# pySTEPS/pysteps

Measured on AMD Instinct MI355X. Metric: Mpixels*leadsteps/s (LK+semilag) at 4096x4096 fp32, higher is better.
Workload: dtype f32

## Files before the change

### pysteps_amd/csrc/lk.hip

```cpp
#include <algorithm>
#include <cmath>
#include <cstring>
#include <functional>
#include <vector>

#include "common.h"

#pragma clang fp contract(off)

namespace psh {
namespace {

enum Stat : int {
  kMinAll = 0,
  kNanCount,
  kMaxAll,
  kMinFeat,
  kMaxFeat,
  kEigMax,
  kNumStats = 8
};

constexpr int kRedBlocks = 1024;

// ... 333 lines not shown
    unsigned char t[4], f[4];
#pragma unroll
    for (int j = 0; j < 4; ++j) {
      const size_t p = i + j;
      float v = p < npx ? clean[p] : fill;
      const bool ok = isfinite(v);
      if (!ok) v = fill;
      t[j] = quantise(v, fill, hi);
      f[j] = quantise((ok && p >= first_feature_px) ? v : fill, flo, fhi);
    }
    if (i + 3 < npx && (npx & 3) == 0) {
      *reinterpret_cast<uchar4 *>(trk + i) = make_uchar4(t[0], t[1], t[2], t[3]);
      if (feat) *reinterpret_cast<uchar4 *>(feat + i) = make_uchar4(f[0], f[1], f[2], f[3]);
    } else {
      for (int j = 0; j < 4 && i + j < npx; ++j) {
        trk[i + j] = t[j];
        if (feat) feat[i + j] = f[j];
      }
    }
  }
}

constexpr int kU8Rows = 4;
template <bool VEC>
__global__ __launch_bounds__(256) void lk_to_u8_bits(const float *__restrict__ img,
                                                     const unsigned long long *__restrict__ keepbits, int nstrips,
                                                     int m, int n, int buffer_mask, float *__restrict__ stats,
                                                     unsigned char *__restrict__ trk, unsigned char *__restrict__ feat,
                                                     const unsigned *__restrict__ slots) {
  const float fill = stats[kMinAll], hi = slots_max(slots, kSlMaxAll);
  const float flo = slots_min(slots, kSlMinFeat), fhi = slots_max(slots, kSlMaxFeat);
  if (blockIdx.x == 0 && blockIdx.y == 0 && threadIdx.x == 0) {
    stats[kMaxAll] = hi;
    stats[kMinFeat] = flo;
    stats[kMaxFeat] = fhi;
  }
  const int first_row = buffer_mask > 0 ? (stats[kNanCount] > 0.f ? 2 : 1) : 0;
  const bool same_scale = flo == fill && fhi == hi;
  const int x = (blockIdx.x * 256 + threadIdx.x) * 4;
  const int y0 = blockIdx.y * kU8Rows;
  if (x >= n) return;
  const int strip = x / kOpenColsW, shift = x - strip * kOpenColsW + 2;
  float v[kU8Rows][4];
  unsigned long long w[kU8Rows];
#pragma unroll
  for (int r = 0; r < kU8Rows; ++r) {
    const int y = min(y0 + r, m - 1);
    const float *row = img + static_cast<size_t>(y) * n + x;
    w[r] = keepbits[static_cast<size_t>(y) * nstrips + strip];
    if (VEC) {
      const float4 q = *reinterpret_cast<const float4 *>(row);
      v[r][0] = q.x, v[r][1] = q.y, v[r][2] = q.z, v[r][3] = q.w;
    } else {
#pragma unroll
      for (int j = 0; j < 4; ++j) v[r][j] = x + j < n ? row[j] : 0.f;
    }
  }
#pragma unroll
  for (int r = 0; r < kU8Rows; ++r) {
    const int y = y0 + r;
    if (y >= m) break;
    const unsigned keep = static_cast<unsigned>(w[r] >> shift);
    unsigned t = 0, f = 0;
#pragma unroll
    for (int j = 0; j < 4; ++j) {
      const bool k = (keep >> j) & 1u;
      const float val = k ? v[r][j] : fill;
      t |= static_cast<unsigned>(quantise(val, fill, hi)) << (8 * j);
      if (!same_scale) f |= static_cast<unsigned>(quantise(y >= first_row ? val : fill, flo, fhi)) << (8 * j);
    }
    if (same_scale) f = y >= first_row ? t : 0u;
    const size_t at = static_cast<size_t>(y) * n + x;
    if (VEC) {
      *reinterpret_cast<unsigned *>(trk + at) = t;
      if (feat) *reinterpret_cast<unsigned *>(feat + at) = f;
    } else {
#pragma unroll
      for (int j = 0; j < 4; ++j) {
        if (x + j >= n) break;
        trk[at + j] = static_cast<unsigned char>(t >> (8 * j));
        if (feat) feat[at + j] = static_cast<unsigned char>(f >> (8 * j));
      }
    }
  }
}

__device__ __forceinline__ double wave_min_d(double v) {
#pragma unroll
  for (int d = 32; d >= 1; d >>= 1) v = fmin(v, __shfl_xor(v, d));
  return v;
}
__device__ __forceinline__ double wave_max_d(double v) {
#pragma unroll
  for (int d = 32; d >= 1; d >>= 1) v = fmax(v, __shfl_xor(v, d));
  return v;
}

__global__ __launch_bounds__(256) void lk_stats1_f64(const double *__restrict__ img, size_t npx,
                                                     double *__restrict__ partial) {
  double mn = INFINITY, bad = 0.0;
  const size_t stride = static_cast<size_t>(gridDim.x) * blockDim.x;
  for (size_t i = static_cast<size_t>(blockIdx.x) * blockDim.x + threadIdx.x; i < npx; i += stride) {
    const double v = img[i];
    const bool fin = isfinite(v);
    mn = fmin(mn, fin ? v : INFINITY);
    bad += fin ? 0.0 : 1.0;
  }
  __shared__ double s[2][4];
  mn = wave_min_d(mn);
#pragma unroll
  for (int d = 32; d >= 1; d >>= 1) bad += __shfl_xor(bad, d);
  if ((threadIdx.x & 63) == 0) {
    s[0][threadIdx.x >> 6] = mn;
    s[1][threadIdx.x >> 6] = bad;
  }
  __syncthreads();
  if (threadIdx.x == 0) {
    partial[blockIdx.x] = fmin(fmin(s[0][0], s[0][1]), fmin(s[0][2], s[0][3]));
    partial[gridDim.x + blockIdx.x] = s[1][0] + s[1][1] + s[1][2] + s[1][3];
  }
}

__global__ __launch_bounds__(kFinalThreads) void lk_final_f64(const double *__restrict__ partial, int nb, int what,
                                                             float *__restrict__ stats, double *__restrict__ dstats) {
  __shared__ double sm[3][16];
  double a = what == 0 ? INFINITY : -INFINITY, b = what == 0 ? 0.0 : INFINITY, c = -INFINITY;
  for (int i = threadIdx.x; i < nb; i += blockDim.x) {
    if (what == 0) {
      a = fmin(a, partial[i]);
      b += partial[nb + i];
    } else {
      a = fmax(a, partial[i]);
      b = fmin(b, partial[nb + i]);
      c = fmax(c, partial[2 * nb + i]);
    }
  }
  if (what == 0) {
    a = wave_min_d(a);
#pragma unroll
    for (int d = 32; d >= 1; d >>= 1) b += __shfl_xor(b, d);
  } else {
    a = wave_max_d(a);
    b = wave_min_d(b);
    c = wave_max_d(c);
  }
  const int wave = threadIdx.x >> 6, nwaves = blockDim.x >> 6;
  if ((threadIdx.x & 63) == 0) {
    sm[0][wave] = a;
    sm[1][wave] = b;
    sm[2][wave] = c;
  }
  __syncthreads();
  if (threadIdx.x == 0) {
    for (int w = 1; w < nwaves; ++w) {
      if (what == 0) {
        a = fmin(a, sm[0][w]);
        b += sm[1][w];
      } else {
        a = fmax(a, sm[0][w]);
        b = fmin(b, sm[1][w]);
        c = fmax(c, sm[2][w]);
      }
    }
    if (what == 0) {
      dstats[0] = a;
      stats[kMinAll] = static_cast<float>(a);
      stats[kNanCount] = static_cast<float>(b);
    } else {
      dstats[1] = a;
      dstats[2] = b;
      dstats[3] = c;
      stats[kMaxAll] = static_cast<float>(a);
      stats[kMinFeat] = static_cast<float>(b);
      stats[kMaxFeat] = static_cast<float>(c);
    }
  }
}

__global__ __launch_bounds__(256) void lk_open_bits_f64(const double *__restrict__ img, int m, int n,
                                                        int size_opening, int buffer_mask,
                                                        const float *__restrict__ stats,
                                                        const double *__restrict__ dstats,
                                                        float *__restrict__ clean32, double *__restrict__ clean64,
                                                        double *__restrict__ partial) {
  __shared__ double red[3][4];
  const double mn = dstats[0];
  const int lane = threadIdx.x & 63, wave = threadIdx.x >> 6;
  const int x = blockIdx.x * kOpenColsW - 2 + lane;
  const int yb = blockIdx.y * kOpenRowsWG + wave * kOpenRowsW;
  const bool col_in = x >= 0 && x < n;
  constexpr int kLoad = kOpenRowsW + 4;
  double v[kLoad];
#pragma unroll
  for (int q = 0; q < kLoad; ++q) {
    const int y = yb - 2 + q;
    v[q] = (col_in && y >= 0 && y < m) ? img[static_cast<size_t>(y) * n + x] : 0.0;
  }
  unsigned long long A[kLoad], F[kLoad];
#pragma unroll
  for (int q = 0; q < kLoad; ++q) {
    const int y = yb - 2 + q;
    const bool row_in = y >= 0 && y < m;
    F[q] = __ballot(row_in && col_in && isfinite(v[q]) && v[q] > mn);
    A[q] = F[q] | __ballot(!(row_in && col_in));
  }
  unsigned long long E[kLoad];
#pragma unroll
  for (int q = 1; q < kLoad - 1; ++q) E[q] = F[q] & (A[q] << 1) & (A[q] >> 1) & A[q - 1] & A[q + 1];
  double mx_all = -INFINITY, mn_feat = INFINITY, mx_feat = -INFINITY;
  const int first_row = buffer_mask > 0 ? (stats[kNanCount] > 0.f ? 2 : 1) : 0;
  const bool writer = lane >= 2 && lane < 2 + kOpenColsW && col_in;
#pragma unroll
  for (int q = 2; q < kLoad - 2; ++q) {
    const int y = yb - 2 + q;
    if (y >= m) break;
    const unsigned long long O = E[q] | (E[q] << 1) | (E[q] >> 1) | E[q - 1] | E[q + 1];
    double val = v[q];
    if (size_opening > 0 && ((F[q] >> lane) & 1ull) && !((O >> lane) & 1ull)) val = mn;
    if (writer) {
      if (isfinite(val)) {
        mx_all = fmax(mx_all, val);
        if (y >= first_row) {
          mn_feat = fmin(mn_feat, val);
          mx_feat = fmax(mx_feat, val);
        }
      }
      clean64[static_cast<size_t>(y) * n + x] = val;
      clean32[static_cast<size_t>(y) * n + x] = static_cast<float>(val);
    }
  }
  mx_all = wave_max_d(mx_all);
  mn_feat = wave_min_d(mn_feat);
  mx_feat = wave_max_d(mx_feat);
  if (lane == 0) {
    red[0][wave] = mx_all;
    red[1][wave] = mn_feat;
    red[2][wave] = mx_feat;
  }
  __syncthreads();
  if (threadIdx.x == 0) {
    const int b = blockIdx.y * gridDim.x + blockIdx.x, nb = gridDim.x * gridDim.y;
    partial[b] = fmax(fmax(red[0][0], red[0][1]), fmax(red[0][2], red[0][3]));
    partial[nb + b] = fmin(fmin(red[1][0], red[1][1]), fmin(red[1][2], red[1][3]));
    partial[2 * nb + b] = fmax(fmax(red[2][0], red[2][1]), fmax(red[2][2], red[2][3]));
  }
}

__device__ __forceinline__ unsigned char quantise_f64(double v, double lo, double hi) {
  const double s = (hi - lo) > 1e-8 ? (v - lo) / (hi - lo) * 255.0 : v - lo;
  return static_cast<unsigned char>(static_cast<int>(s));
}

__global__ __launch_bounds__(256) void lk_to_u8_f64(const double *__restrict__ clean, int m, int n, int buffer_mask,
                                                    const float *__restrict__ stats,
                                                    const double *__restrict__ dstats,
                                                    unsigned char *__restrict__ trk, unsigned char *__restrict__ feat) {
  const double fill = dstats[0], hi = dstats[1], flo = dstats[2], fhi = dstats[3];
  const int first_row = buffer_mask > 0 ? (stats[kNanCount] > 0.f ? 2 : 1) : 0;
  const size_t npx = static_cast<size_t>(m) * n;
  const size_t first_feature_px = static_cast<size_t>(first_row) * n;
  const size_t stride = static_cast<size_t>(gridDim.x) * blockDim.x;
  for (size_t p = static_cast<size_t>(blockIdx.x) * blockDim.x + threadIdx.x; p < npx; p += stride) {
    double v = clean[p];
    const bool ok = isfinite(v);
    if (!ok) v = fill;
    trk[p] = quantise_f64(v, fill, hi);
    if (feat) feat[p] = quantise_f64((ok && p >= first_feature_px) ? v : fill, flo, fhi);
  }
}

constexpr int kMaxBlockR = 3;

__device__ __forceinline__ bool px_allowed(const float *__restrict__ clean, int m, int n, int x,
                                           int y, int bm, bool any_nan) {
  if (!any_nan) return true;
  if (bm <= 0) return isfinite(clean[static_cast<size_t>(y) * n + x]);
  const int a = bm / 2;
  for (int j = 0; j < bm; ++j) {
    const int yy = y + j - a;
    if (yy < 0 || yy >= m) continue;
    for (int i = 0; i < bm; ++i) {
      const int xx = x + i - a;
      if (xx < 0 || xx >= n) continue;
      if (!isfinite(clean[static_cast<size_t>(yy) * n + xx])) return false;
    }
  }
  return true;
}

__device__ __forceinline__ float next_lane_f(float v) {
  return __int_as_float(__builtin_amdgcn_update_dpp(0, __float_as_int(v), 0x130 , 0xf, 0xf, true));
}
__device__ __forceinline__ double next_lane_d(double v) {
  const int lo = __builtin_amdgcn_update_dpp(0, __double2loint(v), 0x130, 0xf, 0xf, true);
  const int hi = __builtin_amdgcn_update_dpp(0, __double2hiint(v), 0x130, 0xf, 0xf, true);
  return __hiloint2double(hi, lo);
}
__device__ __forceinline__ bool walk_mirrored(int i, int n) {
  if (i >= 0 && i + 1 < n) return false;
  return reflect101(i + 1, n) != reflect101(reflect101(i, n) + 1, n);
}

constexpr int crn_cols(int block_size) { return 64 - 2 * (block_size / 2 + 1); }

template <int BS, int ROWS>
__global__ __launch_bounds__(256) void lk_corner_response_cols(
    const unsigned char *__restrict__ u8, const float *__restrict__ clean, int m, int n,
    int buffer_mask, const float *__restrict__ stats, float *__restrict__ eig,
    float *__restrict__ partial, Band band, unsigned *__restrict__ slots, int *__restrict__ zero_a, int count_a,
    int *__restrict__ zero_b, int count_b) {
  constexpr int r = BS / 2, H = r + 1, W = crn_cols(BS);
  if (blockIdx.x == 0 && blockIdx.y == 0) {
    for (int i = threadIdx.x; i < count_a; i += 256) zero_a[i] = 0;
    for (int i = threadIdx.x; i < count_b; i += 256) zero_b[i] = 0;
  }
  __shared__ float red[4];
  const int lane = threadIdx.x & 63, wave = __builtin_amdgcn_readfirstlane(threadIdx.x >> 6);
  const int x0 = blockIdx.x * W;
  const int yb = (blockIdx.y * 4 + wave) * ROWS;
  float best = 0.f;
  if (yb < m) {
    const float s = 1.0f / (4.0f * static_cast<float>(BS) * 255.0f), s2 = 2.f * s;
    const int xl = x0 - H + lane;
    const bool neg_x = walk_mirrored(xl + 1, n);
    const float sx = neg_x ? -s : s, sx2 = neg_x ? -s2 : s2;
    const unsigned char *col = u8 + reflect101(xl, n);
    const bool few_rows = m < 2 * H + 2;
    auto row_of = [&](int y) -> int {
      if (few_rows) return reflect101(y, m);
      y = y < 0 ? -y : y;
      return y >= m ? 2 * m - 2 - y : y;
    };
    auto load_row = [&](int i) -> int { return col[static_cast<size_t>(row_of(yb - H + i)) * n]; };
    auto row_terms = [&](int raw, float &hd, float &g) {
      const float a = static_cast<float>(raw);
      const float c = next_lane_f(a);
      const float b = next_lane_f(c);
      hd = b - a;
      g = (a + b) * s + c * s2;
    };
    const bool any_nan = stats[kNanCount] > 0.f;
    const int x = x0 + lane;
    const bool writer = lane < W && x < n;
    const int rows_out = min(ROWS, m - yb);
    const int last_p = rows_out + BS - 1;
    double ring[3][BS], V[3] = {0.0, 0.0, 0.0};
#pragma unroll
    for (int j = 0; j < BS; ++j) ring[0][j] = ring[1][j] = ring[2][j] = 0.0;
    int raw[BS];
    const int raw0 = load_row(0), raw1 = load_row(1);
#pragma unroll
    for (int j = 0; j < BS; ++j) raw[j] = load_row(2 + j);
    float hd_m, hd_0, g_m, g_0;
    row_terms(raw0, hd_m, g_m);
    row_terms(raw1, hd_0, g_0);
    for (int base = 1; base <= last_p; base += BS) {
      int nxt[BS];
#pragma unroll
      for (int j = 0; j < BS; ++j) nxt[j] = load_row(base + BS + 1 + j);
#pragma unroll
      for (int j = 0; j < BS; ++j) {
        const int p = base + j;
        if (p > last_p) break;
        constexpr int kRingBase = 1;
        const int slot = (kRingBase + j) % BS;
        float hd_p, g_p;
        row_terms(raw[j], hd_p, g_p);
        const float dx = (hd_m + hd_p) * sx + hd_0 * sx2;
        float dy = g_p - g_m;
        const int y_seq = yb - H + p;
        const bool row_mirrored = few_rows ? walk_mirrored(y_seq, m) : (y_seq < 0 || y_seq >= m);
        const unsigned row_sign = row_mirrored ? 0x80000000u : 0u;
        dy = __uint_as_float(__float_as_uint(dy) ^ row_sign);
        const double pxx = static_cast<double>(dx * dx), pxy = static_cast<double>(dx * dy);
        const double pyy = static_cast<double>(dy * dy);
        V[0] += pxx - ring[0][slot];
        V[1] += pxy - ring[1][slot];
        V[2] += pyy - ring[2][slot];
        ring[0][slot] = pxx;
        ring[1][slot] = pxy;
        ring[2][slot] = pyy;
        hd_m = hd_0;
        hd_0 = hd_p;
        g_m = g_0;
        g_0 = g_p;
        if (p >= BS) {
          double w0 = V[0], w1 = V[1], w2 = V[2];
          double t0 = V[0], t1 = V[1], t2 = V[2];
#pragma unroll
          for (int c = 0; c < 2 * r; ++c) {
            t0 = next_lane_d(t0);
            t1 = next_lane_d(t1);
            t2 = next_lane_d(t2);
            w0 += t0;
            w1 += t1;
            w2 += t2;
          }
          const int y = yb + p - BS;
          if (writer) {
            const float a = static_cast<float>(w0) * 0.5f, b = static_cast<float>(w1);
            const float c = static_cast<float>(w2) * 0.5f;
            const float e = (a + c) - sqrtf((a - c) * (a - c) + b * b);
            eig[static_cast<size_t>(y) * n + x] = e;
            if (y >= band.lo && y < band.hi && px_allowed(clean, m, n, x, y, buffer_mask, any_nan))
              best = fmaxf(best, fmaxf(e, 0.f));
          }
        }
      }
#pragma unroll
      for (int j = 0; j < BS; ++j) raw[j] = nxt[j];
    }
  }
  best = wave_max(best);
  if (lane == 0) red[wave] = best;
  __syncthreads();
  if (threadIdx.x == 0) {
    const int b = blockIdx.y * gridDim.x + blockIdx.x;
    const float b_max = fmaxf(fmaxf(red[0], red[1]), fmaxf(red[2], red[3]));
    if (slots) {
      slot_max(slots, kSlEig, b, b_max);
    } else {
      partial[b] = b_max;
    }
  }
}

constexpr int kNmsKeys = 64;

using CornerKeyT = unsigned long long;
__device__ __forceinline__ CornerKeyT nms_key(float val, unsigned addr) {
  return (static_cast<CornerKeyT>(__float_as_uint(val)) << 32) | addr;
}
__device__ __forceinline__ float prev_lane_f(float v) {
  return __int_as_float(__builtin_amdgcn_update_dpp(0, __float_as_int(v), 0x138 , 0xf, 0xf, true));
}

template <int BS, int ROWS>
__global__ __launch_bounds__(256) void lk_corner_response_nms(
    const unsigned char *__restrict__ u8, const float *__restrict__ clean, int m, int n, int buffer_mask,
    const float *__restrict__ stats, float quality, CornerKeyT *__restrict__ out, int cap, Band band,
    unsigned *__restrict__ slots, int *__restrict__ zero_b, int count_b) {
  constexpr int r = BS / 2, H = r + 1, W = crn_cols(BS);
  if (blockIdx.x == 0 && blockIdx.y == 0)
    for (int i = threadIdx.x; i < count_b; i += 256) zero_b[i] = 0;
  __shared__ float red[4];
  const int lane = threadIdx.x & 63, wave = __builtin_amdgcn_readfirstlane(threadIdx.x >> 6);
  int *over_count = reinterpret_cast<int *>(slots + kSlCand * kSlots);
  const int fixed_total = static_cast<int>(gridDim.x * gridDim.y) * 4 * kNmsKeys;
  const int my_slots = (static_cast<int>(blockIdx.y * gridDim.x + blockIdx.x) * 4 + wave) * kNmsKeys;
  const int x0 = blockIdx.x * (W - 2) - 1;
  const int yj = (blockIdx.y * 4 + wave) * ROWS;
  const int yb = yj - 1;
  float best = 0.f;
  float known = fmaxf(slots_max(slots, kSlEig), 0.f);
  int held = 0;
  if (yj < m) {
    const float s = 1.0f / (4.0f * static_cast<float>(BS) * 255.0f), s2 = 2.f * s;
    const int xl = x0 - H + lane;
    const bool neg_x = walk_mirrored(xl + 1, n);
    const float sx = neg_x ? -s : s, sx2 = neg_x ? -s2 : s2;
    const unsigned char *col = u8 + reflect101(xl, n);
    const bool few_rows = m < 2 * H + 4;
    auto row_of = [&](int y) -> int {
      if (few_rows) return reflect101(y, m);
      y = y < 0 ? -y : y;
      return y >= m ? 2 * m - 2 - y : y;
    };
    auto load_row = [&](int i) -> int { return col[static_cast<size_t>(row_of(yb - H + i)) * n]; };
    auto row_terms = [&](int raw, float &hd, float &g) {
      const float a = static_cast<float>(raw);
      const float c = next_lane_f(a);
      const float b = next_lane_f(c);
      hd = b - a;
      g = (a + b) * s + c * s2;
    };
    const bool any_nan = stats[kNanCount] > 0.f;
    const int x = x0 + lane;
    const bool in_image_col = lane < W && x >= 0 && x < n;
    const bool judged_col = lane >= 1 && lane < W - 1 && x >= 1 && x < n - 1;
    const int rows_e = min(ROWS + 2, m - yb);
    const int last_p = rows_e + BS - 1;
    double ring[3][BS], V[3] = {0.0, 0.0, 0.0};
#pragma unroll
    for (int j = 0; j < BS; ++j) ring[0][j] = ring[1][j] = ring[2][j] = 0.0;
    int raw[BS];
    const int raw0 = load_row(0), raw1 = load_row(1);
#pragma unroll
    for (int j = 0; j < BS; ++j) raw[j] = load_row(2 + j);
    float hd_m, hd_0, g_m, g_0;
    row_terms(raw0, hd_m, g_m);
    row_terms(raw1, hd_0, g_0);
    float c1 = 0.f, h1 = 0.f, t1 = 0.f, t2 = 0.f;
    for (int base = 1; base <= last_p; base += BS) {
      int nxt[BS];
#pragma unroll
      for (int j = 0; j < BS; ++j) nxt[j] = load_row(base + BS + 1 + j);
#pragma unroll
      for (int j = 0; j < BS; ++j) {
        const int p = base + j;
        if (p > last_p) break;
        constexpr int kRingBase = 1;
        const int slot = (kRingBase + j) % BS;
        float hd_p, g_p;
        row_terms(raw[j], hd_p, g_p);
        const float dx = (hd_m + hd_p) * sx + hd_0 * sx2;
        float dy = g_p - g_m;
        const int y_seq = yb - H + p;
        const bool row_mirrored = few_rows ? walk_mirrored(y_seq, m) : (y_seq < 0 || y_seq >= m);
        const unsigned row_sign = row_mirrored ? 0x80000000u : 0u;
        dy = __uint_as_float(__float_as_uint(dy) ^ row_sign);
        const double pxx = static_cast<double>(dx * dx), pxy = static_cast<double>(dx * dy);
        const double pyy = static_cast<double>(dy * dy);
        V[0] += pxx - ring[0][slot];
        V[1] += pxy - ring[1][slot];
        V[2] += pyy - ring[2][slot];
        ring[0][slot] = pxx;
        ring[1][slot] = pxy;
        ring[2][slot] = pyy;
        hd_m = hd_0;
        hd_0 = hd_p;
        g_m = g_0;
        g_0 = g_p;
        if (p >= BS) {
          double w0 = V[0], w1 = V[1], w2 = V[2];
          double q0 = V[0], q1 = V[1], q2 = V[2];
#pragma unroll
          for (int c = 0; c < 2 * r; ++c) {
            q0 = next_lane_d(q0);
            q1 = next_lane_d(q1);
            q2 = next_lane_d(q2);
            w0 += q0;
            w1 += q1;
            w2 += q2;
          }
          const int y = yb + p - BS;
          const float a = static_cast<float>(w0) * 0.5f, b = static_cast<float>(w1);
          const float c = static_cast<float>(w2) * 0.5f;
          const float e = (a + c) - sqrtf((a - c) * (a - c) + b * b);
          if (in_image_col && y >= 0 && y >= band.lo && y < band.hi && px_allowed(clean, m, n, x, y, buffer_mask, any_nan))
            best = fmaxf(best, fmaxf(e, 0.f));
          if ((p & 7) == 0) known = fmaxf(known, wave_max(best));
          const float h0 = fmaxf(prev_lane_f(e), next_lane_f(e)), t0 = fmaxf(e, h0);
          const int yr = y - 1;
          if (p >= BS + 2 && yr >= yj) {
            bool keep = judged_col && yr >= 1 && yr < m - 1 && yr >= band.lo && yr < band.hi;
            keep = keep && c1 > 0.f && c1 > known * quality;
            keep = keep && !(fmaxf(h1, fmaxf(t2, t0)) > c1);
            keep = keep && px_allowed(clean, m, n, x, yr, buffer_mask, any_nan);
            const unsigned long long mask = __ballot(keep);
            if (mask != 0ull) {
              const int cnt = __popcll(mask);
              int at = held + __popcll(mask & ((1ull << lane) - 1ull));
              if (held + cnt > kNmsKeys) {
                int base = 0;
                const int spill = held + cnt - max(held, kNmsKeys);
                if (lane == 0) base = atomicAdd(over_count, spill);
                base = __shfl(base, 0);
                if (at >= kNmsKeys) at = fixed_total + base + (at - max(held, kNmsKeys)) - my_slots;
              }
              if (keep && my_slots + at < cap) out[my_slots + at] = nms_key(c1, static_cast<unsigned>(yr + band.y_org) * n + x);
              held += cnt;
            }
          }
          t2 = t1;
          t1 = t0;
          h1 = h0;
          c1 = e;
        }
      }
#pragma unroll
      for (int j = 0; j < BS; ++j) raw[j] = nxt[j];
    }
  }
  for (int i = min(held, kNmsKeys) + lane; i < kNmsKeys; i += 64)
    if (my_slots + i < cap) out[my_slots + i] = 0ull;
  best = wave_max(best);
  if (lane == 0) red[wave] = best;
  __syncthreads();
  if (threadIdx.x == 0)
    slot_max(slots, kSlEig, blockIdx.y * gridDim.x + blockIdx.x, fmaxf(fmaxf(red[0], red[1]), fmaxf(red[2], red[3])));
}

__global__ __launch_bounds__(kFinalThreads) void lk_max_final(const float *__restrict__ partial,
                                                              int nb, float *__restrict__ stats,
                                                              int slot, int *__restrict__ zero_a, int count_a,
                                                              int *__restrict__ zero_b, int count_b) {
  __shared__ float smem[16];
  for (int i = threadIdx.x; i < count_a; i += blockDim.x) zero_a[i] = 0;
  for (int i = threadIdx.x; i < count_b; i += blockDim.x) zero_b[i] = 0;
  float a = -INFINITY;
  for (int i = threadIdx.x; i < nb; i += blockDim.x) a = fmaxf(a, partial[i]);
  a = block_reduce<Red::kMax>(a, smem);
  if (threadIdx.x == 0) stats[slot] = a;
}

using CornerKey = unsigned long long;
__host__ __device__ inline CornerKey make_corner_key(float val, unsigned addr) {
#if defined(__HIP_DEVICE_COMPILE__)
  const unsigned bits = __float_as_uint(val);
#else
  unsigned bits;
  std::memcpy(&bits, &val, sizeof(bits));
#endif
  return (static_cast<CornerKey>(bits) << 32) | addr;
}

#ifndef PSH_SEL_WAVES
#define PSH_SEL_WAVES 4
#endif
#ifndef PSH_SEL_GROUPS
#define PSH_SEL_GROUPS 4
#endif
#ifndef PSH_SEL_WIDE
#define PSH_SEL_WIDE 1
#endif
constexpr int kSelWaves = PSH_SEL_WAVES;
constexpr int kSelGroups = PSH_SEL_GROUPS;
constexpr bool kSelWide = PSH_SEL_WIDE != 0;
constexpr int kSelCols = 62;
constexpr int kSelWgRows = kSelWide ? 16 * kSelGroups : 16 * kSelGroups * kSelWaves;
constexpr int kSelWgCols = kSelWide ? kSelCols * kSelWaves : kSelCols;

__global__ __launch_bounds__(64 * kSelWaves) void lk_corner_select(const float *__restrict__ eig,
                                                        const float *__restrict__ clean, int m,
                                                        int n, int buffer_mask, float quality,
                                                        float *__restrict__ stats,
                                                        CornerKey *__restrict__ out, int cap,
                                                        int *__restrict__ count, Band band,
                                                        const unsigned *__restrict__ slots) {
  constexpr int kRows = 16;
  __shared__ unsigned long long s_mask[kSelWaves][kSelGroups * kRows];
  __shared__ int wave_count[kSelWaves];
  __shared__ int block_base;
  const int lane = threadIdx.x & 63, wave = threadIdx.x >> 6;
  const int x = (kSelWide ? (blockIdx.x * kSelWaves + wave) : blockIdx.x) * kSelCols - 1 + lane, xc = x + 1;
  const int y_wave = (kSelWide ? blockIdx.y : (blockIdx.y * kSelWaves + wave)) * (kSelGroups * kRows);
  const float eig_max = slots ? slots_max(slots, kSlEig) : stats[kEigMax];
  if (slots && blockIdx.x == 0 && blockIdx.y == 0 && threadIdx.x == 0) stats[kEigMax] = eig_max;
  const float thr = eig_max * quality;
  const bool any_nan = stats[kNanCount] > 0.f;
  const bool col_in = x >= 0 && x < n;
  const bool col_ok = lane < kSelCols && xc >= 1 && xc < n - 1;
  int mine = 0;
  for (int g = 0; g < kSelGroups; ++g) {
    const int y_first = y_wave + g * kRows;
    if (y_first >= m) {
      if (lane < kRows) s_mask[wave][g * kRows + lane] = 0ull;
      continue;
    }
    float v[kRows + 2], m3[kRows + 2], hmax[kRows + 2];
#pragma unroll
    for (int q = 0; q < kRows + 2; ++q) {
      const int y = y_first - 1 + q;
      v[q] = (col_in && y >= 0 && y < m) ? eig[static_cast<size_t>(y) * n + x] : 0.f;
    }
#pragma unroll
    for (int q = 0; q < kRows + 2; ++q) {
      const float left = v[q], centre = next_lane_f(left), right = next_lane_f(centre);
      hmax[q] = fmaxf(left, right);
      m3[q] = fmaxf(centre, hmax[q]);
      v[q] = centre;
    }
#pragma unroll
    for (int r = 0; r < kRows; ++r) {
      const int yr = y_first + r;
      const float c = v[r + 1];
      bool keep = col_ok && yr >= 1 && yr < m - 1 && yr >= band.lo && yr < band.hi;
      keep = keep && c > thr && c != 0.f;
      keep = keep && !(fmaxf(hmax[r + 1], fmaxf(m3[r], m3[r + 2])) > c);
      keep = keep && px_allowed(clean, m, n, xc, yr, buffer_mask, any_nan);
      const unsigned long long mask = __ballot(keep);
      if (lane == 0) s_mask[wave][g * kRows + r] = mask;
      mine += __popcll(mask);
    }
  }
  if (lane == 0) wave_count[wave] = mine;
  __syncthreads();
  if (threadIdx.x == 0) {
    int total = 0;
    for (int w = 0; w < kSelWaves; ++w) total += wave_count[w];
    block_base = total > 0 ? atomicAdd(count, total) : 0;
  }
  __syncthreads();
  int pos = block_base;
  for (int w = 0; w < wave; ++w) pos += wave_count[w];
  if (mine == 0) return;
  for (int r = 0; r < kSelGroups * kRows; ++r) {
    const unsigned long long mask = s_mask[wave][r];
    if (mask == 0ull) continue;
    const int y = y_wave + r;
    if ((mask >> lane) & 1ull) {
      const int at = pos + __popcll(mask & ((1ull << lane) - 1ull));
      if (at < cap)
        out[at] = make_corner_key(eig[static_cast<size_t>(y) * n + xc], static_cast<unsigned>(y + band.y_org) * n + xc);
    }
    pos += __popcll(mask);
  }
}

constexpr int kPyrRows = 8;

struct PyrPair {
  const unsigned char *src[2];
  unsigned char *dst[2];
};

template <bool FAST>
__device__ __forceinline__ void pyr_rows(const unsigned char *__restrict__ src, unsigned char *__restrict__ dst, int m,
                                         int n, int om, int on, int ox, int oy0, int wx, const int (&off)[11]) {
  auto window = [&](const unsigned char *row) -> uint4 {
    if (FAST) return *reinterpret_cast<const uint4 *>(row + wx);
    unsigned w[4] = {0u, 0u, 0u, 0u};
#pragma unroll
    for (int k = 0; k < 11; ++k) w[(k + 2) >> 2] |= static_cast<unsigned>(row[off[k]]) << (8 * ((k + 2) & 3));
    return make_uint4(w[0], w[1], w[2], w[3]);
  };
  auto hrow = [&](const uint4 d, int h[4]) {
    const unsigned w[4] = {d.x, d.y, d.z, d.w};
    auto b = [&](int k) -> int { return static_cast<int>((w[(k + 2) >> 2] >> (8 * ((k + 2) & 3))) & 0xffu); };
#pragma unroll
    for (int j = 0; j < 4; ++j) h[j] = b(2 * j) + b(2 * j + 4) + 4 * (b(2 * j + 1) + b(2 * j + 3)) + 6 * b(2 * j + 2);
  };
  auto row_ptr = [&](int y) { return src + static_cast<size_t>(reflect101(y, m)) * n; };
  const bool store4 = (on & 3) == 0 && (reinterpret_cast<uintptr_t>(dst) & 3) == 0 && ox + 3 < on;
  constexpr int kHalf = kPyrRows / 2, kIn = 2 * kHalf + 3;
  int h[kIn][4];
#pragma unroll
  for (int half = 0; half < 2; ++half) {
    const int oyh = oy0 + half * kHalf;
    if (oyh >= om) break;
    const int keep = half == 0 ? 0 : 3;
    if (half != 0) {
#pragma unroll
      for (int q = 0; q < 3; ++q)
#pragma unroll
        for (int j = 0; j < 4; ++j) h[q][j] = h[kIn - 3 + q][j];
    }
    uint4 d[kIn];
#pragma unroll
    for (int q = keep; q < kIn; ++q) d[q] = window(row_ptr(2 * oyh - 2 + q));
#pragma unroll
    for (int q = keep; q < kIn; ++q) hrow(d[q], h[q]);
#pragma unroll
    for (int i = 0; i < kHalf; ++i) {
      const int oy = oyh + i;
      if (oy >= om) break;
      unsigned packed = 0;
#pragma unroll
      for (int j = 0; j < 4; ++j) {
        const int v = h[2 * i][j] + 4 * h[2 * i + 1][j] + 6 * h[2 * i + 2][j] + 4 * h[2 * i + 3][j] + h[2 * i + 4][j];
        packed |= static_cast<unsigned>((v + 128) >> 8) << (8 * j);
      }
      unsigned char *out = dst + static_cast<size_t>(oy) * on + ox;
      if (store4) {
        *reinterpret_cast<unsigned *>(out) = packed;
      } else {
#pragma unroll
        for (int j = 0; j < 4; ++j)
          if (ox + j < on) out[j] = static_cast<unsigned char>(packed >> (8 * j));
      }
    }
  }
}

__global__ __launch_bounds__(256) void lk_pyrdown(PyrPair pair, int m, int n, int om, int on) {
  const unsigned char *__restrict__ src = pair.src[blockIdx.z];
  unsigned char *__restrict__ dst = pair.dst[blockIdx.z];
  const int lane = threadIdx.x & 63, wave = __builtin_amdgcn_readfirstlane(threadIdx.x >> 6);
  const int ox = (blockIdx.x * 64 + lane) * 4;
  const int oy0 = (blockIdx.y * 4 + wave) * kPyrRows;
  if (oy0 >= om) return;
  const int wx = 2 * ox - 4;
  const bool rows_aligned = (n & 3) == 0 && (reinterpret_cast<uintptr_t>(src) & 3) == 0;
  const bool fast = rows_aligned && wx >= 0 && wx + 16 <= n;
  int off[11] = {0, 0, 0, 0, 0, 0, 0, 0, 0, 0, 0};
  if (fast) {
    pyr_rows<true>(src, dst, m, n, om, on, ox, oy0, wx, off);
  } else if (ox < on) {
#pragma unroll
    for (int k = 0; k < 11; ++k) {
      int i = wx + 2 + k;
      if (n < 16) {
        i = reflect101(i, n);
      } else {
        i = i < 0 ? -i : i;
        i = i >= n ? 2 * n - 2 - i : i;
        i = min(max(i, 0), n - 1);
      }
      off[k] = i;
    }
    pyr_rows<false>(src, dst, m, n, om, on, ox, oy0, wx, off);
  }
}

__global__ __launch_bounds__(256) void lk_scharr(const unsigned char *__restrict__ src, int m,
                                                 int n, short2 *__restrict__ dst) {
  constexpr int TX = 64, TY = 4;
  __shared__ short tile[TY + 2][TX + 2];
  const int x0 = blockIdx.x * TX, y0 = blockIdx.y * TY;
  const int tid = threadIdx.x;
  for (int i = tid; i < (TY + 2) * (TX + 2); i += 256) {
    const int ly = i / (TX + 2), lx = i % (TX + 2);
    const int y = reflect101(y0 + ly - 1, m), x = reflect101(x0 + lx - 1, n);
    tile[ly][lx] = src[static_cast<size_t>(y) * n + x];
  }
  __syncthreads();
  const int lx = tid % TX + 1, ly = tid / TX + 1;
  const int x = x0 + lx - 1, y = y0 + ly - 1;
  if (x < n && y < m) {
    const int t0l = (tile[ly - 1][lx - 1] + tile[ly + 1][lx - 1]) * 3 + tile[ly][lx - 1] * 10;
    const int t0r = (tile[ly - 1][lx + 1] + tile[ly + 1][lx + 1]) * 3 + tile[ly][lx + 1] * 10;
    const int t1l = tile[ly + 1][lx - 1] - tile[ly - 1][lx - 1];
    const int t1c = tile[ly + 1][lx] - tile[ly - 1][lx];
    const int t1r = tile[ly + 1][lx + 1] - tile[ly - 1][lx + 1];
    dst[static_cast<size_t>(y) * n + x] =
        make_short2(static_cast<short>(t0r - t0l), static_cast<short>((t1r + t1l) * 3 + t1c * 10));
  }
}

constexpr int kMaxLevels = 8;
constexpr int kMaxWin = 64;

struct PyrLevel {
  const unsigned char *I, *J;
  const short2 *dI;
  int rows, cols;
  int vlo = -(1 << 30), vhi = 1 << 30;
  int row_org = 0, rows_stored = 1 << 30;
};
__device__ __forceinline__ size_t stored_row(const PyrLevel &L, int y) {
  return static_cast<size_t>(min(max(y - L.row_org, 0), L.rows_stored - 1));
}
struct Pyramid {
  PyrLevel lv[kMaxLevels];
  int top;
};

__device__ __forceinline__ long long wave_sum_i64(long long v) {
#pragma unroll
  for (int d = 32; d >= 1; d >>= 1) v += __shfl_xor(v, d);
  return v;
}

__device__ __forceinline__ int wave_sum_dpp_i32(int v) {
#define PSH_SUM_STEP(CTRL, ROWMASK) v += __builtin_amdgcn_update_dpp(0, v, CTRL, ROWMASK, 0xf, false);
  PSH_SUM_STEP(0xB1, 0xf)
  PSH_SUM_STEP(0x4E, 0xf)
  PSH_SUM_STEP(0x141, 0xf)
  PSH_SUM_STEP(0x140, 0xf)
  PSH_SUM_STEP(0x142, 0xa)
  PSH_SUM_STEP(0x143, 0xc)
#undef PSH_SUM_STEP
  return __builtin_amdgcn_readlane(v, 63);
}
__device__ __forceinline__ long long wave_sum_split_i64(int v) {
  const int lo = wave_sum_dpp_i32(v & 0xffff), hi = wave_sum_dpp_i32(v >> 16);
  return (static_cast<long long>(hi) << 16) + lo;
}

__device__ __forceinline__ void lk_weights(float a, float b, int &w00, int &w01, int &w10, int &w11) {
  const float s = 16384.f;
  w00 = static_cast<int>(rintf((1.f - a) * (1.f - b) * s));
  w01 = static_cast<int>(rintf(a * (1.f - b) * s));
  w10 = static_cast<int>(rintf((1.f - a) * b * s));
  w11 = 16384 - w00 - w01 - w10;
}

__device__ __forceinline__ int descale(int v, int n) { return (v + (1 << (n - 1))) >> n; }
__device__ __forceinline__ int bilin24(int a, int b, int c, int d, int w00, int w01, int w10, int w11) {
  return __mul24(a, w00) + __mul24(b, w01) + __mul24(c, w10) + __mul24(d, w11);
}

template <int kPer>
__global__ __launch_bounds__(256) void lk_track(Pyramid pyr, const float2 *__restrict__ pts,
                                                int npts, const int *__restrict__ npts_dev, int win_w,
                                                int win_h, int max_count, float eps2, float min_eig_thr,
                                                float2 *__restrict__ next_pts,
                                                unsigned char *__restrict__ status) {
  __shared__ short sI[kMaxWin * kMaxWin];
  __shared__ short sGx[kMaxWin * kMaxWin];
  __shared__ short sGy[kMaxWin * kMaxWin];
  __shared__ long long red[3][4];
  const int p = blockIdx.x;
  if (npts_dev) npts = min(npts, *npts_dev);
  if (p >= npts) return;
  const int tid = threadIdx.x, wave = tid >> 6, lane = tid & 63;
  const int area = win_w * win_h;
  const float half_x = (win_w - 1) * 0.5f, half_y = (win_h - 1) * 0.5f;
  const float2 pt = pts[p];
  float nx = 0.f, ny = 0.f;
  bool ok = true, suspect = false;
  int wxs[kPer], wys[kPer];
#pragma unroll
  for (int q = 0; q < kPer; ++q) {
    const int i = min(tid + 256 * q, area - 1);
    wys[q] = i / win_w;
    wxs[q] = i - wys[q] * win_w;
  }

  for (int level = pyr.top; level >= 0; --level) {
    const PyrLevel L = pyr.lv[level];
    const float scale = 1.f / static_cast<float>(1 << level);
    float px = pt.x * scale, py = pt.y * scale;
    if (level == pyr.top) {
      nx = px;
      ny = py;
    } else {
      nx *= 2.f;
      ny *= 2.f;
    }
    px -= half_x;
    py -= half_y;
    const int ipx = static_cast<int>(floorf(px)), ipy = static_cast<int>(floorf(py));
    if (ipy - 1 < L.vlo || ipy + win_h + 2 > L.vhi) suspect = true;
    if (ipx < -win_w || ipx >= L.cols || ipy < -win_h || ipy >= L.rows) {
      if (level == 0) ok = false;
      continue;
    }
    int w00, w01, w10, w11;
    lk_weights(px - static_cast<float>(ipx), py - static_cast<float>(ipy), w00, w01, w10, w11);
    int s11 = 0, s12 = 0, s22 = 0;
    __syncthreads();
#pragma unroll
    for (int q = 0; q < kPer; ++q) {
      const int i = tid + 256 * q;
      if (i < area) {
        const int x = ipx + wxs[q], y = ipy + wys[q];
        const int xa = reflect101(x, L.cols), xb = reflect101(x + 1, L.cols);
        const int ya = reflect101(y, L.rows), yb = reflect101(y + 1, L.rows);
        const unsigned char *ra = L.I + stored_row(L, ya) * L.cols;
        const unsigned char *rb = L.I + stored_row(L, yb) * L.cols;
        const int ival = descale(ra[xa] * w00 + ra[xb] * w01 + rb[xa] * w10 + rb[xb] * w11, 14 - 5);
        const bool x_in0 = x >= 0 && x < L.cols, x_in1 = x + 1 >= 0 && x + 1 < L.cols;
        const bool y_in0 = y >= 0 && y < L.rows, y_in1 = y + 1 >= 0 && y + 1 < L.rows;
        const short2 z = make_short2(0, 0);
        const short2 g00 = (x_in0 && y_in0) ? L.dI[stored_row(L, y) * L.cols + x] : z;
        const short2 g01 = (x_in1 && y_in0) ? L.dI[stored_row(L, y) * L.cols + x + 1] : z;
        const short2 g10 = (x_in0 && y_in1) ? L.dI[stored_row(L, y + 1) * L.cols + x] : z;
        const short2 g11 = (x_in1 && y_in1) ? L.dI[stored_row(L, y + 1) * L.cols + x + 1] : z;
        const int gx = descale(g00.x * w00 + g01.x * w01 + g10.x * w10 + g11.x * w11, 14);
        const int gy = descale(g00.y * w00 + g01.y * w01 + g10.y * w10 + g11.y * w11, 14);
        sI[i] = static_cast<short>(ival);
        sGx[i] = static_cast<short>(gx);
        sGy[i] = static_cast<short>(gy);
        s11 += gx * gx;
        s12 += gx * gy;
        s22 += gy * gy;
      }
    }
    long long a11 = s11, a12 = s12, a22 = s22;
    a11 = wave_sum_i64(a11);
    a12 = wave_sum_i64(a12);
    a22 = wave_sum_i64(a22);
    if (lane == 0) {
      red[0][wave] = a11;
      red[1][wave] = a12;
      red[2][wave] = a22;
// ... 1275 lines not shown
```

Baseline: 277,600.

## Skip corner-response work over flat row runs and empty selection groups

Result: no change. 279,400 (median of 6 runs) (+0.6%).

```diff
diff --git a/pysteps_amd/csrc/lk.hip b/pysteps_amd/csrc/lk.hip
--- a/pysteps_amd/csrc/lk.hip
+++ b/pysteps_amd/csrc/lk.hip
@@ -659,6 +659,30 @@
 }
 
 constexpr int crn_cols(int block_size) { return 64 - 2 * (block_size / 2 + 1); }
+
+struct FlatRun {
+  int run = 0, value = -1;
+  __device__ __forceinline__ void note(int raw) {
+    const int first = __builtin_amdgcn_readfirstlane(raw);
+    const bool is_flat = __ballot(raw != first) == 0ull;
+    run = is_flat ? (first == value ? run + 1 : 1) : 0;
+    value = first;
+  }
+  template <int BS>
+  __device__ __forceinline__ void note_group(const int (&raw)[BS]) {
+    const int first = __builtin_amdgcn_readfirstlane(raw[BS - 1]);
+    if (__ballot(raw[BS - 1] != first) != 0ull) {
+      run = 0;
+      return;
+    }
+#pragma unroll
+    for (int j = 0; j < BS; ++j) note(raw[j]);
+  }
+};
+template <int BS>
+__device__ __forceinline__ bool flat_group_skippable(int base, int run_before, int run_after) {
+  return run_after >= run_before + BS && run_before >= 2 && (base == 1 || run_before >= BS + 2);
+}
 
 template <int BS, int ROWS>
 __global__ __launch_bounds__(256) void lk_corner_response_cols(
@@ -711,10 +735,29 @@
     float hd_m, hd_0, g_m, g_0;
     row_terms(raw0, hd_m, g_m);
     row_terms(raw1, hd_0, g_0);
+    FlatRun flat;
+    flat.note(raw0);
+    flat.note(raw1);
     for (int base = 1; base <= last_p; base += BS) {
       int nxt[BS];
 #pragma unroll
       for (int j = 0; j < BS; ++j) nxt[j] = load_row(base + BS + 1 + j);
+      const int run_before = flat.run;
+      flat.note_group(raw);
+      if (!few_rows && flat_group_skippable<BS>(base, run_before, flat.run)) {
+#pragma unroll
+        for (int j = 0; j < BS; ++j) {
+          const int p = base + j;
+          if (p > last_p) break;
+          if (p >= BS && writer) eig[static_cast<size_t>(yb + p - BS) * n + x] = 0.f;
+        }
+        row_terms(raw[BS - 1], hd_0, g_0);
+        hd_m = hd_0;
+        g_m = g_0;
+#pragma unroll
+        for (int j = 0; j < BS; ++j) raw[j] = nxt[j];
+        continue;
+      }
 #pragma unroll
       for (int j = 0; j < BS; ++j) {
         const int p = base + j;
@@ -848,10 +891,59 @@
     row_terms(raw0, hd_m, g_m);
     row_terms(raw1, hd_0, g_0);
     float c1 = 0.f, h1 = 0.f, t1 = 0.f, t2 = 0.f;
+    auto judge_row = [&](int p, float e) {
+      const int y = yb + p - BS;
+      if ((p & 7) == 0) known = fmaxf(known, wave_max(best));
+      const float h0 = fmaxf(prev_lane_f(e), next_lane_f(e)), t0 = fmaxf(e, h0);
+      const int yr = y - 1;
+      if (p >= BS + 2 && yr >= yj) {
+        bool keep = judged_col && yr >= 1 && yr < m - 1 && yr >= band.lo && yr < band.hi;
+        keep = keep && c1 > 0.f && c1 > known * quality;
+        keep = keep && !(fmaxf(h1, fmaxf(t2, t0)) > c1);
+        keep = keep && px_allowed(clean, m, n, x, yr, buffer_mask, any_nan);
+        const unsigned long long mask = __ballot(keep);
+        if (mask != 0ull) {
+          const int cnt = __popcll(mask);
+          int at = held + __popcll(mask & ((1ull << lane) - 1ull));
+          if (held + cnt > kNmsKeys) {
+            int base = 0;
+            const int spill = held + cnt - max(held, kNmsKeys);
+            if (lane == 0) base = atomicAdd(over_count, spill);
+            base = __shfl(base, 0);
+            if (at >= kNmsKeys) at = fixed_total + base + (at - max(held, kNmsKeys)) - my_slots;
+          }
+          if (keep && my_slots + at < cap) out[my_slots + at] = nms_key(c1, static_cast<unsigned>(yr + band.y_org) * n + x);
+          held += cnt;
+        }
+      }
+      t2 = t1;
+      t1 = t0;
+      h1 = h0;
+      c1 = e;
+    };
+    FlatRun flat;
+    flat.note(raw0);
+    flat.note(raw1);
     for (int base = 1; base <= last_p; base += BS) {
       int nxt[BS];
 #pragma unroll
       for (int j = 0; j < BS; ++j) nxt[j] = load_row(base + BS + 1 + j);
+      const int run_before = flat.run;
+      flat.note_group(raw);
+      if (!few_rows && flat_group_skippable<BS>(base, run_before, flat.run)) {
+#pragma unroll
+        for (int j = 0; j < BS; ++j) {
+          const int p = base + j;
+          if (p > last_p) break;
+          if (p >= BS) judge_row(p, 0.f);
+        }
+        row_terms(raw[BS - 1], hd_0, g_0);
+        hd_m = hd_0;
+        g_m = g_0;
+#pragma unroll
+        for (int j = 0; j < BS; ++j) raw[j] = nxt[j];
+        continue;
+      }
 #pragma unroll
       for (int j = 0; j < BS; ++j) {
         const int p = base + j;
@@ -896,33 +988,7 @@
           const float e = (a + c) - sqrtf((a - c) * (a - c) + b * b);
           if (in_image_col && y >= 0 && y >= band.lo && y < band.hi && px_allowed(clean, m, n, x, y, buffer_mask, any_nan))
             best = fmaxf(best, fmaxf(e, 0.f));
-          if ((p & 7) == 0) known = fmaxf(known, wave_max(best));
-          const float h0 = fmaxf(prev_lane_f(e), next_lane_f(e)), t0 = fmaxf(e, h0);
-          const int yr = y - 1;
-          if (p >= BS + 2 && yr >= yj) {
-            bool keep = judged_col && yr >= 1 && yr < m - 1 && yr >= band.lo && yr < band.hi;
-            keep = keep && c1 > 0.f && c1 > known * quality;
-            keep = keep && !(fmaxf(h1, fmaxf(t2, t0)) > c1);
-            keep = keep && px_allowed(clean, m, n, x, yr, buffer_mask, any_nan);
-            const unsigned long long mask = __ballot(keep);
-            if (mask != 0ull) {
-              const int cnt = __popcll(mask);
-              int at = held + __popcll(mask & ((1ull << lane) - 1ull));
-              if (held + cnt > kNmsKeys) {
-                int base = 0;
-                const int spill = held + cnt - max(held, kNmsKeys);
-                if (lane == 0) base = atomicAdd(over_count, spill);
-                base = __shfl(base, 0);
-                if (at >= kNmsKeys) at = fixed_total + base + (at - max(held, kNmsKeys)) - my_slots;
-              }
-              if (keep && my_slots + at < cap) out[my_slots + at] = nms_key(c1, static_cast<unsigned>(yr + band.y_org) * n + x);
-              held += cnt;
-            }
-          }
-          t2 = t1;
-          t1 = t0;
-          h1 = h0;
-          c1 = e;
+          judge_row(p, e);
         }
       }
 #pragma unroll
@@ -1010,6 +1076,14 @@
     for (int q = 0; q < kRows + 2; ++q) {
       const int y = y_first - 1 + q;
       v[q] = (col_in && y >= 0 && y < m) ? eig[static_cast<size_t>(y) * n + x] : 0.f;
+    }
+    float top = v[0];
+#pragma unroll
+    for (int q = 1; q + 1 < kRows + 2; q += 2) top = fmaxf(fmaxf(top, v[q]), v[q + 1]);
+    top = fmaxf(top, v[kRows + 1]);
+    if (__ballot(top > thr) == 0ull) {
+      if (lane < kRows) s_mask[wave][g * kRows + lane] = 0ull;
+      continue;
     }
 #pragma unroll
     for (int q = 0; q < kRows + 2; ++q) {
```
